# duxfrederic/lightcurver

Measured on AMD Instinct MI355X. Metric: cutouts/sec (PSF-fit + joint forward-model iter), 32x32 & 64x64 stamps, higher is better.
Workload: dtype f32

## Files before the change

lightcurver_amd/csrc/psf_kernels.h:

```cpp
#pragma once
#include <type_traits>
#include <utility>

#include "lc_common.h"
#include "starlet_device.h"

#ifndef LC_XPOLL_SLEEP
#define LC_XPOLL_SLEEP 2
#endif
#ifndef LC_P5_AHEAD
#define LC_P5_AHEAD 1
#endif
#ifndef LC_STARLET_LIVE_ADDR
#define LC_STARLET_LIVE_ADDR 1
#endif
namespace lc {
constexpr int kXFlagStride = 16;

#ifdef LC_STAMPS
__device__ long long g_stamps[128];
#define LC_STAMP(k)                                                      \
  do {                                                                   \
    if ((blockIdx.x == 0 || blockIdx.x == 8) && threadIdx.x == 0 && it == A.n_iter - 1)  \
      g_stamps[(k) + (blockIdx.x == 8 ? 64 : 0)] = clock64();            \
  } while (0)
#else
#define LC_STAMP(k) do {} while (0)
#endif


struct PsfArgs {
  int F, S, n_iter, t0, hist_stride, mode;
  const float *data, *wgt;
  const float *W;
  const float *norms;
  const float *Tm;
  float *B, *mB, *sB;
  float *stars, *stars_m, *stars_s;
  float *hist;
  float *qscratch;
  float *out_loss, *out_chi2, *out_gstars, *out_ggrid, *out_gT, *out_model;
  float lam_sc, lam_hf;
  lc_adabelief_cfg ab;
  float *xch;
  int *xflags, *xabort;
  int launch_seq, heal, force_abort_it;
  const float *bkB, *bkmB, *bksB, *bkstars, *bkstars_m, *bkstars_s;
  int *heal_count;
  const float *ext_grad;
  const float *sched;
  float *B1, *mB1, *sB1;
  int xcd_fast;
};

typedef float lc_v4f __attribute__((ext_vector_type(4)));
__device__ __forceinline__ void store_sc1_x4(float *p, lc_v4f v) {
  asm volatile("global_store_dwordx4 %0, %1, off sc1\n\ts_nop 2" ::"v"(p), "v"(v) : "memory");
}
__device__ __forceinline__ void store_plain_x4(float *p, lc_v4f v) {
  asm volatile("global_store_dwordx4 %0, %1, off\n\ts_nop 2" ::"v"(p), "v"(v) : "memory");
}
__device__ __forceinline__ void store_sc1_f(float *p, float v) {
  asm volatile("global_store_dword %0, %1, off sc1" ::"v"(p), "v"(v) : "memory");
}
__device__ __forceinline__ void load_sc1_2x4(const float *p, lc_v4f &a, lc_v4f &b) {
  asm volatile("global_load_dwordx4 %0, %2, off sc1\n\tglobal_load_dwordx4 %1, %2, off offset:16 sc1\n\ts_waitcnt vmcnt(0)"
               : "=&v"(a), "=&v"(b)
               : "v"(p)
               : "memory");
}
__device__ __forceinline__ void load_sc1_2x4_1(const float *p, lc_v4f &a, lc_v4f &b, const float *ps, float &s) {
  asm volatile("global_load_dword %2, %4, off sc1\n\tglobal_load_dwordx4 %0, %3, off sc1\n\tglobal_load_dwordx4 %1, %3, off offset:16 sc1\n\ts_waitcnt vmcnt(0)"
               : "=&v"(a), "=&v"(b), "=&v"(s)
               : "v"(p), "v"(ps)
               : "memory");
}
__device__ __forceinline__ void load_sc1_x4(const float *p, lc_v4f &a) {
  asm volatile("global_load_dwordx4 %0, %1, off sc1\n\ts_waitcnt vmcnt(0)" : "=&v"(a) : "v"(p) : "memory");
}
__device__ __forceinline__ float load_sc1_f(const float *p) {
  float v;
  asm volatile("global_load_dword %0, %1, off sc1\n\ts_waitcnt vmcnt(0)" : "=&v"(v) : "v"(p) : "memory");
  return v;
}


template <int N_, int SS_, int PX_, int SG_, bool WC_ = false, int JB_ = 8>
struct PsfCfg {
  static constexpr int N = N_, SS = SS_, PX = PX_, SG = SG_;
  static constexpr bool WC = WC_;
  static constexpr int n = N / SS;
  static constexpr int NTHR = N * N / PX;
  static constexpr int NW = (NTHR + kWave - 1) / kWave;
  static constexpr int NT = ntaps(SS);
  static constexpr int J = ilog2(N);
  static constexpr int LR = 8;
  static constexpr int LC = (JB_ * (N_ / SS_) / 4 >= 64) ? 4 : 2;
  static constexpr int LA = LC;
  static constexpr int TS = N + 1;
  static constexpr int RS = n + 1;
  static constexpr int OFF_T = 0;
  static constexpr int SZ_T = WC_ ? N * (N + 2 * (N / 4 + 10) + 1) : N * TS;
  static constexpr int OFF_R = OFF_T + SZ_T;
  static constexpr int SZ_R2 = SG * n * TS;
  static constexpr int VS = WC_ ? n + 3 : RS, VO = WC_ ? 1 : 0;
  static constexpr int SZ_V = SG * N * VS;
  static constexpr int JB = JB_;
  static constexpr int AP = N / 4 + 10;
  static constexpr int TSA = N + 2 * AP + 1;
  static constexpr int APR = AP / SS + 2;
  static constexpr int JBP = JB + 1;
  static constexpr int WSZ = JB * TSA + (n + 2 * APR) * JBP;
  static constexpr int SZ_VR = (SZ_V > StarletLds<N>::FLOATS) ? SZ_V : StarletLds<N>::FLOATS;
  static constexpr int OFF_WSC = OFF_R + SZ_VR;
  static constexpr int SZ_R = WC ? (SZ_VR + NW * WSZ) : ((2 * SZ_R2 > SZ_V) ? 2 * SZ_R2 : SZ_V);
  static constexpr int OFF_RES = OFF_R + SZ_R;
  static constexpr int SZ_RES = WC ? 0 : SG * n * n;
  static constexpr int OFF_TAPS = OFF_RES + SZ_RES;
  static constexpr int NTP = NT + 3;
  static constexpr int SZ_TAPS = (16 * 4 * NTP + 1) / 2 * 2 + 16 * 2 * NT * 2;
  static constexpr int OFF_TAPP = OFF_TAPS + (16 * 4 * NTP + 1) / 2 * 2;
  static constexpr int OFF_RED = OFF_TAPS + SZ_TAPS;
  static constexpr int IPS = n * n / LC;
  static constexpr int IPS_PAD = (IPS + kWave - 1) / kWave * kWave;
  static constexpr int SLOTS = IPS_PAD / kWave;
  static constexpr int SZ_REDX = 16 * NW;
  static constexpr int SZ_RED = (WC ? 16 * (n / JB) * 5 : SG * SLOTS * 5) + SZ_REDX + NW + 8;
  static constexpr int OFF_REDX = OFF_RED + (WC ? 16 * (n / JB) * 5 : SG * SLOTS * 5);
  static constexpr int OFF_REDW = OFF_REDX + SZ_REDX;
  static constexpr int OFF_STAR = OFF_RED + SZ_RED;
  static constexpr int MAXS = 16;
  static constexpr int SZ_STAR = MAXS * 20 + 16;
  static constexpr int LDS_FLOATS = OFF_STAR + SZ_STAR;
  static_assert(WC || StarletLds<N>::FLOATS <= SZ_T + SZ_R + SZ_RES, "starlet ping-pong buffers must fit over T + R + RES");
  static_assert(PX % SS == 0 && N % PX == 0 && n % LR == 0 && n % LC == 0 && n % LA == 0 && n % JB == 0, "tiling");
  static_assert(LDS_FLOATS * 4 <= 163840, "LDS");
  static_assert(OFF_TAPP % 2 == 0, "tap pairs are read as 64-bit words");
  static_assert(NTHR <= 1024 && NTHR % kWave == 0, "threads");
  static_assert(!WC_ || PX_ <= 8, "the WC layout keeps the pixel state in registers");
};


template <int SS, int NT>
__device__ inline void tap_entry(float delta, int k, float &tap, float &dtap, int &bq) {
  const int o = (int)nearbyintf(delta);
  const int base = o - kRg - (SS - 1);
  int q = base / SS;
  if (q * SS > base) --q;
  bq = q;
  const int m = q * SS + k;
  const float inv_s2 = 1.0f / (kSigmaG * kSigmaG);
  const float nrm = 0.3989422804014327f / kSigmaG;
  float a = 0.f, d = 0.f;
#pragma unroll
  for (int dv = 0; dv < SS; ++dv) {
    const int t = m + dv;
    if (t >= o - kRg && t <= o + kRg) {
      const float x = (float)t - delta;
      const float p = nrm * expf(-0.5f * x * x * inv_s2);
      a += p;
      d += p * x * inv_s2;
    }
  }
  tap = a;
  dtap = d;
}

template <class C, bool SPLIT = false>
__global__ __launch_bounds__(C::NTHR) void psf_fit_kernel(PsfArgs A) {
  constexpr int N = C::N, SS = C::SS, PX = C::PX, SG = C::SG, n = C::n, NT = C::NT, J = C::J;
  constexpr int NTHR = C::NTHR, TS = C::TS, RS = C::RS, LR = C::LR, LC = C::LC, LA = C::LA;
  extern __shared__ __align__(16) float lds[];
  float *T = lds + C::OFF_T;
  float *R2t = lds + C::OFF_R;
  float *R2xt = R2t + C::SZ_R2;
  float *V = lds + C::OFF_R;
  float *RES = lds + C::OFF_RES;
  float *TAPS = lds + C::OFF_TAPS + 1;
  constexpr int NTP = C::NTP;
  lc_v2f *TAPP = (lc_v2f *)(lds + C::OFF_TAPP);
  float *REDX = lds + C::OFF_REDX;
  float *RED = lds + C::OFF_RED;
  float *REDW = lds + C::OFF_REDW;
  float *SCAL = REDW + C::NW;
  float *SP = lds + C::OFF_STAR;
  float *SGR = SP + C::MAXS * 4;
  float *SM = SGR + C::MAXS * 5;
  float *SV = SM + C::MAXS * 4;
  int *BQ = (int *)(SV + C::MAXS * 4);

  int f = blockIdx.x, role = 0;
  if constexpr (SPLIT) {
    f = ((int)blockIdx.x >> 4) * 8 + ((int)blockIdx.x & 7);
    role = ((int)blockIdx.x >> 3) & 1;
    if (f >= A.F) return;
  }
  const bool conv_role = !SPLIT || role == 0, starlet_role = !SPLIT || role == 1;
  const int my_xcc = SPLIT ? (int)(__builtin_amdgcn_s_getreg(20 | (3 << 11)) & 15u) : 0;
  int same_xcd = 0;
  const int tid0 = threadIdx.x;
  const int S = A.S;

  const float *dataf = A.data + (size_t)f * S * n * n;
  const float *wgtf = A.wgt + (size_t)f * S * n * n;

  if constexpr (!SPLIT) {
    if (A.heal) {
      if (__hip_atomic_load(A.xabort, __ATOMIC_RELAXED, __HIP_MEMORY_SCOPE_AGENT) != A.launch_seq) return;
      const size_t o = (size_t)f * N * N;
      for (int i = tid0; i < N * N; i += NTHR) {
        A.B[o + i] = A.bkB[o + i];
        A.mB[o + i] = A.bkmB[o + i];
        A.sB[o + i] = A.bksB[o + i];
      }
      if (tid0 < S * 4) {
        A.stars[(size_t)f * S * 4 + tid0] = A.bkstars[(size_t)f * S * 4 + tid0];
        A.stars_m[(size_t)f * S * 4 + tid0] = A.bkstars_m[(size_t)f * S * 4 + tid0];
        A.stars_s[(size_t)f * S * 4 + tid0] = A.bkstars_s[(size_t)f * S * 4 + tid0];
      }
      if (f == 0 && tid0 == 0) atomicAdd(A.heal_count, 1);
      __threadfence_block();
      __syncthreads();
    }
  }

  if constexpr (C::WC) {
    for (int i = tid0; i < C::SZ_T; i += NTHR) lds[C::OFF_T + i] = 0.f;
    for (int i = tid0; i < C::NW * C::WSZ; i += NTHR) lds[C::OFF_WSC + i] = 0.f;
  }
  if (tid0 < S * 4) {
    SP[tid0] = A.stars[(size_t)f * S * 4 + tid0];
    SM[tid0] = A.stars_m[(size_t)f * S * 4 + tid0];
    SV[tid0] = A.stars_s[(size_t)f * S * 4 + tid0];
  }
  __syncthreads();

  constexpr bool STATE_REGS = (PX <= 8);
  float *Bg = A.B, *mBg = A.mB, *sBg = A.sB;
  if constexpr (SPLIT && !STATE_REGS) {
    if (role == 1) {
      const size_t g0pix = (size_t)f * N * N + (size_t)(tid0 / (N / PX)) * N + (tid0 % (N / PX)) * PX;
#pragma unroll
      for (int q = 0; q < PX / 4; ++q) {
        ((float4 *)(A.B1 + g0pix))[q] = ((const float4 *)(A.B + g0pix))[q];
        ((float4 *)(A.mB1 + g0pix))[q] = ((const float4 *)(A.mB + g0pix))[q];
        ((float4 *)(A.sB1 + g0pix))[q] = ((const float4 *)(A.sB + g0pix))[q];
      }
      Bg = A.B1;
      mBg = A.mB1;
      sBg = A.sB1;
    }
  }
  float Bp[PX], Mp[PX], Sp_[PX], Tp[PX];
  {
    const size_t g0pix = (size_t)f * N * N + (size_t)(tid0 / (N / PX)) * N + (tid0 % (N / PX)) * PX;
#pragma unroll
    for (int q = 0; q < PX / 4; ++q) {
      if (STATE_REGS) {
        const float4 b = ((const float4 *)(A.B + g0pix))[q], t = ((const float4 *)(A.Tm + g0pix))[q];
        const float4 m = ((const float4 *)(A.mB + g0pix))[q], sv = ((const float4 *)(A.sB + g0pix))[q];
        Bp[4 * q] = b.x; Bp[4 * q + 1] = b.y; Bp[4 * q + 2] = b.z; Bp[4 * q + 3] = b.w;
        Tp[4 * q] = t.x; Tp[4 * q + 1] = t.y; Tp[4 * q + 2] = t.z; Tp[4 * q + 3] = t.w;
        Mp[4 * q] = m.x; Mp[4 * q + 1] = m.y; Mp[4 * q + 2] = m.z; Mp[4 * q + 3] = m.w;
        Sp_[4 * q] = sv.x; Sp_[4 * q + 1] = sv.y; Sp_[4 * q + 2] = sv.z; Sp_[4 * q + 3] = sv.w;
      }
    }
  }

  auto compute_taps = [&](int tid) {
    for (int e = tid; e < S * 2 * NTP; e += NTHR) {
      const int s = e / (2 * NTP), ax = (e / NTP) & 1, k = e % NTP - 1;
      float tap = 0.f, dtap = 0.f;
      int bq = 0;
      const float c_off = (N % 2 == 0) ? 0.5f : 0.0f;
      const float delta = fminf(fmaxf(SS * SP[s * 4 + 1 + ax], -(float)(N / 4)), (float)(N / 4)) + c_off;
      if (k >= 0 && k < NT) tap_entry<SS, NT>(delta, k, tap, dtap, bq);
      TAPS[(s * 4 + 2 * ax) * NTP + k] = tap;
      TAPS[(s * 4 + 2 * ax + 1) * NTP + k] = dtap;
      if (k >= 0 && k < NT) TAPP[(s * 2 + ax) * NT + k] = (lc_v2f){tap, dtap};
      if (k == 0) BQ[s * 2 + ax] = bq;
    }
  };
  auto step_stars = [&](int tid) {
#pragma clang fp contract(off)
    if (tid < S * 3) {
      const float lr = SCAL[0], bc1 = SCAL[1], bc2 = SCAL[2];
      const float b1 = A.ab.b1, b2 = A.ab.b2, eps = A.ab.eps, eps_root = A.ab.eps_root;
      const int s = tid / 3, q = tid % 3;
      const float g = SGR[s * 5 + 1 + q];
      const float mn = b1 * SM[s * 4 + q] + (1.f - b1) * g;
      const float dg = g - mn;
      const float sn = b2 * SV[s * 4 + q] + (1.f - b2) * dg * dg + eps_root;
      SM[s * 4 + q] = mn;
      SV[s * 4 + q] = sn;
      SP[s * 4 + q] -= lr * (mn * bc1) / (sqrtf(sn * bc2) + eps);
    }
  };
  auto update_stars_and_taps = [&](int tid) {
    step_stars(tid);
    __syncthreads();
    compute_taps(tid);
  };
  if (conv_role) compute_taps(tid0);
  for (int it = 0; it < A.n_iter; ++it) {
    const int tglob = A.t0 + it;
    if constexpr (SPLIT) {
      if (A.force_abort_it == it && f == 0 && role == 1) {
        if (tid0 == 0) __hip_atomic_store(A.xabort, A.launch_seq, __ATOMIC_RELAXED, __HIP_MEMORY_SCOPE_AGENT);
        break;
      }
    }
    int tid = tid0;
    LC_LAUNDER(tid);
    const int lane = tid & 63, wid = tid >> 6;
    const int pu = tid / (N / PX);
    const int pv = (tid % (N / PX)) * PX;
    const size_t gpix = (size_t)f * N * N + (size_t)pu * N + pv;
    if (tid < 3 && A.mode == 1) SCAL[tid] = A.sched[3 * tglob + tid];
    LC_STAMP(0);
    float gB[PX];
#pragma unroll
    for (int p = 0; p < PX; ++p) gB[p] = 0.f;
    float tpix[PX];
    if (conv_role) {
    if (C::WC && STATE_REGS) {
#pragma unroll
      for (int p = 0; p < PX; ++p) {
        tpix[p] = Bp[p] + Tp[p];
        T[pu * C::TSA + C::AP + pv + p] = tpix[p];
      }
    } else if (STATE_REGS) {
#pragma unroll
      for (int p = 0; p < PX; ++p) T[pu * TS + pv + p] = Bp[p] + Tp[p];
    } else {
      const float4 *bp = (const float4 *)(Bg + gpix);
      const float4 *tp = (const float4 *)(A.Tm + gpix);
#pragma unroll
      for (int q = 0; q < PX / 4; ++q) {
        const float4 b = bp[q], t = tp[q];
        T[pu * TS + pv + 4 * q + 0] = b.x + t.x;
        T[pu * TS + pv + 4 * q + 1] = b.y + t.y;
        T[pu * TS + pv + 4 * q + 2] = b.z + t.z;
        T[pu * TS + pv + 4 * q + 3] = b.w + t.w;
      }
    }
    if (tid < S * 5) SGR[tid] = 0.f;

    for (int g0 = 0; g0 < S; g0 += SG) {
      __syncthreads();
      LC_STAMP(1 + 5 * (g0 / SG));
      if constexpr (C::WC) {
        constexpr int JB = C::JB, NBLK = n / JB;
        float *wsc = lds + C::OFF_WSC + wid * C::WSZ;
        constexpr int TSA = C::TSA, AP = C::AP, APR = C::APR;
        float *R2w = wsc + AP, *RESw = wsc + JB * TSA + APR * C::JBP;
        int kdone = 0;
        for (int task = wid; task < SG * NBLK; task += C::NW, ++kdone) {
          progress_prio(kdone);
          const int sl = task / NBLK, blk = task % NBLK, s = g0 + sl;
          if (s >= S) continue;
          const int jd0 = blk * JB;
          const float *tx = TAPS + (s * 4 + 0) * NTP, *ty = tx + 2 * NTP, *dty = tx + 3 * NTP;
          const int bqx = BQ[s * 2 + 0], bqy = BQ[s * 2 + 1];
          const float amp = SP[s * 4 + 0], sky = SP[s * 4 + 3];
          constexpr int NI3 = (JB * (n / LC) + 63) / 64;
          float dpre[NI3][LC], wpre[NI3][LC];
#pragma unroll
          for (int i3 = 0; i3 < NI3; ++i3) {
            const int item = lane + 64 * i3;
            const bool ok = item < JB * (n / LC);
            const int jl = item % JB, a0 = (item / JB) * LC;
#pragma unroll
            for (int j = 0; j < LC; ++j) {
              const size_t pix = ok ? ((size_t)s * n * n + (size_t)(a0 + j) * n + jd0 + jl) : 0;
              const float dv = dataf[pix], wv = wgtf[pix];
              dpre[i3][j] = ok ? dv : 0.f;
              wpre[i3][j] = ok ? wv : 0.f;
            }
          }
          LC_STAMP(10);
          {
            const int ws = SS * (jd0 - bqx) - (NT - 1);
            if constexpr (SS == 2) {
              constexpr int NP = (NT + 1) / 2, WL2 = (JB - 1) + NP;
              lc_v2f tr2[NP];
#pragma unroll
              for (int h = 0; h < NP; ++h) tr2[h] = (lc_v2f){tx[NT - 1 - 2 * h], tx[NT - 2 - 2 * h]};
              for (int u = lane; u < N; u += 64) {
                lc_v2f win2[WL2];
                const float *trow = T + u * TSA + AP + ws;
#pragma unroll
                for (int i = 0; i < WL2; ++i) win2[i] = (lc_v2f){trow[2 * i], trow[2 * i + 1]};
                lc_v2f acc[JB];
#pragma unroll
                for (int j = 0; j < JB; ++j) acc[j] = (lc_v2f){0.f, 0.f};
#pragma unroll
                for (int h = 0; h < NP; ++h) {
#pragma unroll
                  for (int j = 0; j < JB; ++j) acc[j] = pk_fma(tr2[h], win2[j + h], acc[j]);
                }
#pragma unroll
                for (int j = 0; j < JB; ++j) R2w[j * TSA + u] = acc[j].x + acc[j].y;
              }
            } else {
              constexpr int WL = SS * (JB - 1) + NT;
              float tk[NT];
#pragma unroll
              for (int k = 0; k < NT; ++k) tk[k] = tx[k];
              for (int u = lane; u < N; u += 64) {
                float win[WL];
                const float *trow = T + u * TSA + AP + ws;
#pragma unroll
                for (int i = 0; i < WL; ++i) win[i] = trow[i];
#pragma unroll
                for (int j = 0; j < JB; ++j) {
                  float acc = 0.f;
#pragma unroll
                  for (int k = 0; k < NT; ++k) acc = fmaf(tk[k], win[SS * j - k + NT - 1], acc);
                  R2w[j * TSA + u] = acc;
                }
              }
            }
          }
          wave_lds_sync();
          LC_STAMP(11);
          float chi = 0.f, ga = 0.f, gy = 0.f, gs = 0.f;
          {
            constexpr int WL = SS * (LC - 1) + NT;
            lc_v2f tyd[NT];
#pragma unroll
            for (int k = 0; k < NT; ++k) tyd[k] = TAPP[(s * 2 + 1) * NT + k];
#pragma unroll
            for (int i3 = 0; i3 < NI3; ++i3) {
              const int item = lane + 64 * i3;
              if (item < JB * (n / LC)) {
                const int jl = item % JB, a0 = (item / JB) * LC;
                const int ws = SS * (a0 - bqy) - (NT - 1);
                float win[WL];
                const float *r2 = R2w + jl * TSA + ws;
#pragma unroll
                for (int i = 0; i < WL; ++i) win[i] = r2[i];
                float lgy = 0.f;
                lc_v2f fvys[LC];
#pragma unroll
                for (int j = 0; j < LC; ++j) fvys[j] = (lc_v2f){0.f, 0.f};
#pragma unroll
                for (int k = 0; k < NT; ++k) {
#pragma unroll
                  for (int j = 0; j < LC; ++j) fvys[j] = pk_fma(tyd[k], pk_bcast(win[SS * j - k + NT - 1]), fvys[j]);
                  if constexpr (LC == 4) asm volatile("" : "+v"(fvys[0]), "+v"(fvys[1]), "+v"(fvys[2]), "+v"(fvys[3]));
                  else asm volatile("" : "+v"(fvys[0]), "+v"(fvys[1]));
                }
#pragma unroll
                for (int j = 0; j < LC; ++j) {
                  const float fv = fvys[j].x, fy = fvys[j].y;
                  const float model = fmaf(amp, fv, sky);
                  const float res = model - dpre[i3][j];
                  const float rw = wpre[i3][j] * res;
                  chi = fmaf(rw, res, chi);
                  ga = fmaf(rw, fv, ga);
                  lgy = fmaf(rw, fy, lgy);
                  gs += rw;
                  RESw[(a0 + j) * C::JBP + jl] = rw;
                  if (A.out_model) A.out_model[(size_t)f * S * n * n + (size_t)s * n * n + (size_t)(a0 + j) * n + jd0 + jl] = model;
                }
                gy += lgy * amp * SS;
              }
            }
          }
          wave_sum4(chi, ga, gy, gs);
          if (lane == 0) {
            float *r = RED + (s * NBLK + blk) * 5;
            r[0] = chi;
            r[1] = ga;
            r[3] = gy;
            r[4] = gs;
          }
          wave_lds_sync();
          LC_STAMP(12);
          {
            constexpr int WI = (SS * LA - 1 + NT - 1) / SS + 1;
            constexpr int NI4 = (JB * (n / LA) + 63) / 64;
            if constexpr (SS == 2) {
              constexpr int NP = (NT + 1) / 2;
              lc_v2f py[NP];
#pragma unroll
              for (int q = 0; q < NP; ++q) py[q] = (lc_v2f){ty[2 * q], ty[2 * q - 1]};
#pragma unroll
              for (int i4 = 0; i4 < NI4; ++i4) {
                const int item = lane + 64 * i4;
                if (item < JB * (n / LA)) {
                  const int jl = item % JB, a0 = (item / JB) * LA;
                  lc_v2f out2[LA];
#pragma unroll
                  for (int h = 0; h < LA; ++h) out2[h] = (lc_v2f){0.f, 0.f};
                  const float *rcol = RESw + (bqy + a0) * C::JBP + jl;
#pragma unroll
                  for (int i = 0; i < WI; ++i) {
                    const lc_v2f rv = pk_bcast(rcol[i * C::JBP]);
#pragma unroll
                    for (int h = 0; h < LA; ++h)
                      if (i - h >= 0 && i - h < NP) out2[h] = pk_fma(py[i - h], rv, out2[h]);
                  }
                  float *vrow = V + (sl * N + SS * a0) * C::VS + C::VO + jd0 + jl;
#pragma unroll
                  for (int h = 0; h < LA; ++h) {
                    vrow[(2 * h) * C::VS] = out2[h].x;
                    vrow[(2 * h + 1) * C::VS] = out2[h].y;
                  }
                  if (jd0 + jl == 0) {
#pragma unroll
                    for (int r = 0; r < SS * LA; ++r) V[(sl * N + SS * a0 + r) * C::VS] = 0.f;
                  }
                  if (jd0 + jl == n - 1) {
#pragma unroll
                    for (int r = 0; r < SS * LA; ++r) V[(sl * N + SS * a0 + r) * C::VS + n + 1] = 0.f;
                  }
                }
              }
            } else {
              float tk[NT];
#pragma unroll
              for (int k = 0; k < NT; ++k) tk[k] = ty[k];
#pragma unroll
              for (int i4 = 0; i4 < NI4; ++i4) {
                const int item = lane + 64 * i4;
                if (item < JB * (n / LA)) {
                  const int jl = item % JB, a0 = (item / JB) * LA;
                  float out[SS * LA];
#pragma unroll
                  for (int r = 0; r < SS * LA; ++r) out[r] = 0.f;
                  const float *rcol = RESw + (bqy + a0) * C::JBP + jl;
#pragma unroll
                  for (int i = 0; i < WI; ++i) {
                    const float rv = rcol[i * C::JBP];
#pragma unroll
                    for (int k = 0; k < NT; ++k) {
                      const int rel = SS * i - k;
                      if (rel >= 0 && rel < SS * LA) out[rel] = fmaf(tk[k], rv, out[rel]);
                    }
                  }
#pragma unroll
                  for (int r = 0; r < SS * LA; ++r) V[(sl * N + SS * a0 + r) * C::VS + C::VO + jd0 + jl] = out[r];
                  if (jd0 + jl == 0) {
#pragma unroll
                    for (int r = 0; r < SS * LA; ++r) V[(sl * N + SS * a0 + r) * C::VS] = 0.f;
                  }
                  if (jd0 + jl == n - 1) {
#pragma unroll
                    for (int r = 0; r < SS * LA; ++r) V[(sl * N + SS * a0 + r) * C::VS + n + 1] = 0.f;
                  }
                }
              }
            }
          }
          wave_lds_sync();
          LC_STAMP(13);
        }
        __builtin_amdgcn_s_setprio(0);
        LC_STAMP(14);
#ifdef LC_STAMPS
        if (blockIdx.x == 0 && lane == 0 && it == A.n_iter - 1) g_stamps[20 + wid] = clock64();
#endif
        __syncthreads();
        LC_STAMP(15);
        if (tid < SG * 5) {
          const int sl = tid / 5, q = tid % 5;
          if (g0 + sl < S && q != 2) {
            float acc = 0.f;
            for (int k = 0; k < NBLK; ++k) acc += RED[((g0 + sl) * NBLK + k) * 5 + q];
            SGR[(g0 + sl) * 5 + q] = acc;
          }
        }
      } else {
      constexpr int NIT3 = (SG * C::IPS_PAD + NTHR - 1) / NTHR;
      float dpre[NIT3][LC], wpre[NIT3][LC];
#pragma unroll
      for (int i3 = 0; i3 < NIT3; ++i3) {
        const int item0 = wid * 64 + i3 * NTHR, item = item0 + lane;
        const int sl = item0 / C::IPS_PAD, within = item % C::IPS_PAD, s = g0 + sl;
        const bool ok = (item0 < SG * C::IPS_PAD) && (s < S) && (within < C::IPS);
        const int jd = within % n, a0 = (within / n) * LC;
#pragma unroll
        for (int j = 0; j < LC; ++j) {
          const size_t pix = ok ? ((size_t)s * n * n + (size_t)(a0 + j) * n + jd) : 0;
          const float dv = dataf[pix], wv = wgtf[pix];
          dpre[i3][j] = ok ? dv : 0.f;
          wpre[i3][j] = ok ? wv : 0.f;
        }
      }
      {
        constexpr int WL = SS * (LR - 1) + NT;
        constexpr int NSTRIP = n / LR;
        for (int item = tid; item < SG * N * NSTRIP; item += NTHR) {
          const int u = item % N, strip = (item / N) % NSTRIP, sl = item / (N * NSTRIP);
          if (g0 + sl >= S) continue;
          const float *tx = TAPS + ((g0 + sl) * 4 + 0) * NTP;
          const int bq = BQ[(g0 + sl) * 2 + 0];
          const int a0 = strip * LR;
          const int ws = SS * (a0 - bq) - (NT - 1);
          float win[WL];
#pragma unroll
          for (int i = 0; i < WL; ++i) {
            const int idx = ws + i;
            const int ci = min(max(idx, 0), N - 1);
            const float v = T[u * TS + ci];
            win[i] = (idx >= 0 && idx < N) ? v : 0.f;
          }
          float tk[NT];
#pragma unroll
          for (int k = 0; k < NT; ++k) tk[k] = tx[k];
#pragma unroll
          for (int j = 0; j < LR; ++j) {
            float acc = 0.f;
#pragma unroll
            for (int k = 0; k < NT; ++k) acc = fmaf(tk[k], win[SS * j - k + NT - 1], acc);
            R2t[(sl * n + a0 + j) * TS + u] = acc;
          }
        }
      }
      __syncthreads();
      LC_STAMP(2 + 5 * (g0 / SG));
      {
        constexpr int WL = SS * (LC - 1) + NT;
        constexpr int NSTRIP = n / LC;
#pragma unroll
        for (int i3 = 0; i3 < NIT3; ++i3) {
          const int item0 = wid * 64 + i3 * NTHR;
          if (item0 >= SG * C::IPS_PAD) break;
          const int item = item0 + lane;
          const int sl = item0 / C::IPS_PAD;
          const int within = item % C::IPS_PAD;
          const int s = g0 + sl;
          float chi = 0.f, ga = 0.f, gx = 0.f, gy = 0.f, gs = 0.f;
          if (s < S && within < C::IPS) {
            const int jd = within % n, strip = within / n;
            const float *ty = TAPS + (s * 4 + 2) * NTP, *dty = ty + NTP;
            const int bq = BQ[s * 2 + 1];
            const int a0 = strip * LC;
            const int ws = SS * (a0 - bq) - (NT - 1);
            const float amp = SP[s * 4 + 0], sky = SP[s * 4 + 3];
            float win[WL];
#pragma unroll
            for (int i = 0; i < WL; ++i) {
              const int idx = ws + i;
              const int ci = min(max(idx, 0), N - 1);
              const bool ok = (idx >= 0 && idx < N);
              const float v = R2t[(sl * n + jd) * TS + ci];
              win[i] = ok ? v : 0.f;
            }
            float tk[NT], dk[NT];
#pragma unroll
            for (int k = 0; k < NT; ++k) {
              tk[k] = ty[k];
              dk[k] = dty[k];
            }
#pragma unroll
            for (int j = 0; j < LC; ++j) {
              float fv = 0.f, fy = 0.f;
#pragma unroll
              for (int k = 0; k < NT; ++k) {
                const float w = win[SS * j - k + NT - 1];
                fv = fmaf(tk[k], w, fv);
                fy = fmaf(dk[k], w, fy);
              }
              const int id = a0 + j;
              const size_t pix = (size_t)s * n * n + (size_t)id * n + jd;
              const float d = dpre[i3][j], w = wpre[i3][j];
              const float model = fmaf(amp, fv, sky);
              const float res = model - d;
              const float rw = w * res;
              chi = fmaf(rw, res, chi);
              ga = fmaf(rw, fv, ga);
              gy = fmaf(rw, fy, gy);
              gs += rw;
              RES[(sl * n + id) * n + jd] = rw;
              if (A.out_model) A.out_model[(size_t)f * S * n * n + pix] = model;
            }
            gy *= amp * SS;
          }
          chi = wave_sum(chi);
          ga = wave_sum(ga);
          gx = wave_sum(gx);
          gy = wave_sum(gy);
          gs = wave_sum(gs);
          if (lane == 0) {
            float *r = RED + (sl * C::SLOTS + (item0 % C::IPS_PAD) / 64) * 5;
            r[0] = chi;
            r[1] = ga;
            r[2] = gx;
            r[3] = gy;
            r[4] = gs;
          }
        }
      }
      __syncthreads();
      LC_STAMP(3 + 5 * (g0 / SG));
      if (tid < SG * 5) {
        const int sl = tid / 5, q = tid % 5;
        if (g0 + sl < S && q != 2) {
          float acc = 0.f;
          for (int k = 0; k < C::SLOTS; ++k) acc += RED[(sl * C::SLOTS + k) * 5 + q];
          SGR[(g0 + sl) * 5 + q] = acc;
        }
      }
      {
        constexpr int WI = (SS * LA - 1 + NT - 1) / SS + 1;
        constexpr int NSTRIP = n / LA;
        for (int item = tid; item < SG * n * NSTRIP; item += NTHR) {
          const int jd = item % n, strip = (item / n) % NSTRIP, sl = item / (n * NSTRIP);
          if (g0 + sl >= S) continue;
          const float *ty = TAPS + ((g0 + sl) * 4 + 2) * NTP;
          const int bq = BQ[(g0 + sl) * 2 + 1];
          const int a0 = strip * LA;
          float tk[NT];
#pragma unroll
          for (int k = 0; k < NT; ++k) tk[k] = ty[k];
          float out[SS * LA];
#pragma unroll
          for (int r = 0; r < SS * LA; ++r) out[r] = 0.f;
#pragma unroll
          for (int i = 0; i < WI; ++i) {
            const int id = i + bq + a0;
            const int ci = min(max(id, 0), n - 1);
            float rv = RES[(sl * n + ci) * n + jd];
            rv = (id >= 0 && id < n) ? rv : 0.f;
#pragma unroll
            for (int k = 0; k < NT; ++k) {
              const int rel = SS * i - k;
              if (rel >= 0 && rel < SS * LA) out[rel] = fmaf(tk[k], rv, out[rel]);
            }
          }
#pragma unroll
          for (int r = 0; r < SS * LA; ++r) V[(sl * N + SS * a0 + r) * RS + jd] = out[r];
        }
      }
      __syncthreads();
      LC_STAMP(4 + 5 * (g0 / SG));
      }
      LC_STAMP(16);
      if constexpr (C::WC) {
        constexpr int WJ = (PX - 1 + NT - 1) / SS + 1;
        constexpr bool AHEAD = SPLIT && PX == 8 && LC_P5_AHEAD;
        if constexpr (AHEAD) {
          static_assert(SG % 8 == 0, "two stars per turn of the loop share a priority step");
          struct P5Ops {
            float vwin[WJ];
            lc_v2f txd[NT];
            float amp;
          };
          auto p5_star = [&](int sl, const P5Ops &use, auto on_the_way) {
            const int s = g0 + sl;
            lc_v2f accp[PX];
#pragma unroll
            for (int p = 0; p < PX; ++p) accp[p] = (lc_v2f){0.f, 0.f};
#pragma unroll
            for (int i = 0; i < WJ; ++i) {
              if (i == 4) on_the_way();
              const lc_v2f vv = pk_bcast(use.vwin[i]);
#pragma unroll
              for (int k = 0; k < NT; ++k) {
                const int rel = SS * i - k;
                if (rel >= 0 && rel < PX) accp[rel] = pk_fma(use.txd[k], vv, accp[rel]);
              }
            }
            float gxs = 0.f;
#pragma unroll
            for (int p = 0; p < PX; ++p) {
              gB[p] = fmaf(use.amp, accp[p].x, gB[p]);
              gxs = fmaf(accp[p].y, tpix[p], gxs);
            }
            gxs = wave_sum(gxs);
            if (lane == 0) REDX[s * C::NW + wid] = gxs;
          };
          auto nothing = [] {};
          auto p5_window = [&](int sl, P5Ops &o, int bq) {
            o.amp = SP[(g0 + sl) * 4 + 0];
            const float *vrow = V + (sl * N + pu) * C::VS + 1;
            const int jd0 = bq + pv / SS;
#pragma unroll
            for (int i = 0; i < WJ; ++i) o.vwin[i] = vrow[min(max(jd0 + i, -1), n)];
            __builtin_amdgcn_sched_barrier(0);
          };
          auto p5_taps = [&](int sl, P5Ops &o) {
            __builtin_amdgcn_sched_barrier(0);
#pragma unroll
            for (int k = 0; k < NT; ++k) o.txd[k] = TAPP[((g0 + sl) * 2 + 0) * NT + k];
            __builtin_amdgcn_sched_barrier(0);
          };
          const int ns = min(SG, S - g0);
          P5Ops opsA, opsB;
          int bqn = BQ[min(g0 + 1, S - 1) * 2 + 0];
          p5_window(0, opsA, BQ[g0 * 2 + 0]);
          p5_taps(0, opsA);
          int sl = 0;
#pragma clang loop unroll(disable)
          while (sl + 1 < ns) {
            progress_prio((4 * sl) / SG);
            const int bqnn = BQ[min(g0 + sl + 2, S - 1) * 2 + 0];
            p5_window(sl + 1, opsB, bqn);
            p5_star(sl, opsA, [&] { p5_taps(sl + 1, opsB); });
            if (sl + 2 >= ns) {
              opsA = opsB;
              sl += 1;
              break;
            }
            bqn = BQ[min(g0 + sl + 3, S - 1) * 2 + 0];
            p5_window(sl + 2, opsA, bqnn);
            p5_star(sl + 1, opsB, [&] { p5_taps(sl + 2, opsA); });
            sl += 2;
          }
          progress_prio((4 * sl) / SG);
          p5_star(sl, opsA, nothing);
        } else {
          for (int sl = 0; sl < SG; ++sl) {
            const int s = g0 + sl;
            if (s >= S) break;
            progress_prio((4 * sl) / SG);
            const int bq = BQ[s * 2 + 0];
            const float amp = SP[s * 4 + 0];
            lc_v2f txd[NT];
#pragma unroll
            for (int k = 0; k < NT; ++k) txd[k] = TAPP[(s * 2 + 0) * NT + k];
            lc_v2f accp[PX];
#pragma unroll
            for (int p = 0; p < PX; ++p) accp[p] = (lc_v2f){0.f, 0.f};
            const float *vrow = V + (sl * N + pu) * C::VS + 1;
            const int jd0 = bq + pv / SS;
            float vwin[WJ];
#pragma unroll
            for (int i = 0; i < WJ; ++i) vwin[i] = vrow[min(max(jd0 + i, -1), n)];
#pragma unroll
            for (int i = 0; i < WJ; ++i) {
              const lc_v2f vv = pk_bcast(vwin[i]);
#pragma unroll
              for (int k = 0; k < NT; ++k) {
                const int rel = SS * i - k;
                if (rel >= 0 && rel < PX) accp[rel] = pk_fma(txd[k], vv, accp[rel]);
              }
            }
            float gxs = 0.f;
#pragma unroll
            for (int p = 0; p < PX; ++p) {
              gB[p] = fmaf(amp, accp[p].x, gB[p]);
              gxs = fmaf(accp[p].y, tpix[p], gxs);
            }
            gxs = wave_sum(gxs);
            if (lane == 0) REDX[s * C::NW + wid] = gxs;
          }
        }
        __builtin_amdgcn_s_setprio(0);
      } else {
        constexpr int WJ = (PX - 1 + NT - 1) / SS + 1;
        for (int sl = 0; sl < SG; ++sl) {
          const int s = g0 + sl;
          if (s >= S) break;
          const float *tx = TAPS + (s * 4 + 0) * NTP, *dtx = tx + NTP;
          const int bq = BQ[s * 2 + 0];
          const float amp = SP[s * 4 + 0];
          float acc[PX], gxs = 0.f;
#pragma unroll
          for (int p = 0; p < PX; ++p) acc[p] = 0.f;
#pragma unroll
          for (int i = 0; i < WJ; ++i) {
            const int jd = i + bq + pv / SS;
            const int ci = min(max(jd, 0), n - 1);
            float vv = V[(sl * N + pu) * RS + ci];
            vv = (jd >= 0 && jd < n) ? vv : 0.f;
            float dsum = 0.f;
#pragma unroll
            for (int k = 0; k < NT; ++k) {
              const int rel = SS * i - k;
              if (rel >= 0 && rel < PX) {
                acc[rel] = fmaf(tx[k], vv, acc[rel]);
                dsum = fmaf(dtx[k], T[pu * TS + pv + rel], dsum);
              }
            }
            gxs = fmaf(vv, dsum, gxs);
          }
#pragma unroll
          for (int p = 0; p < PX; ++p) gB[p] = fmaf(amp, acc[p], gB[p]);
          gxs = wave_sum(gxs);
          if (lane == 0) REDX[s * C::NW + wid] = gxs;
        }
      }
      LC_STAMP(17);
    }
    if (A.ext_grad) {
#pragma unroll
      for (int p = 0; p < PX; ++p) gB[p] += A.ext_grad[gpix + p];
    }
    }
    __syncthreads();
    LC_STAMP(40);
    {
      if (conv_role && tid < S) {
        float acc = 0.f;
#pragma unroll
        for (int w = 0; w < C::NW; ++w) acc += REDX[tid * C::NW + w];
        SGR[tid * 5 + 2] = acc * SP[tid * 4 + 0] * SS;
      }
    }

    if (A.out_gT) {
#pragma unroll
      for (int p = 0; p < PX; ++p) A.out_gT[gpix + p] = gB[p];
    }

    float l1 = 0.f;
    float z[PX];
#pragma unroll
    for (int p = 0; p < PX; ++p) z[p] = 0.f;
    if (starlet_role && (A.lam_sc != 0.f || A.lam_hf != 0.f)) {
      float bpix[PX];
      if (STATE_REGS) {
#pragma unroll
        for (int p = 0; p < PX; ++p) bpix[p] = Bp[p];
      } else {
        const float4 *bp = (const float4 *)(Bg + gpix);
#pragma unroll
        for (int q = 0; q < PX / 4; ++q) {
          const float4 b = bp[q];
          bpix[4 * q] = b.x;
          bpix[4 * q + 1] = b.y;
          bpix[4 * q + 2] = b.z;
          bpix[4 * q + 3] = b.w;
        }
      }
      constexpr bool LIVE_ADDR = SPLIT && STATE_REGS && LC_STARLET_LIVE_ADDR;
      starlet_l1_grad<N, PX, ilog2(N), LIVE_ADDR>(bpix, A.W ? A.W + (size_t)f * J * N * N : nullptr, A.norms,
                                                  A.qscratch + (size_t)f * J * N * N, A.lam_sc, A.lam_hf,
                                                  C::WC ? lds + C::OFF_R : lds, tid, l1, z);
    }
    LC_STAMP(42);
    {
      const float wl = wave_sum(l1);
      if (lane == 0) REDW[wid] = wl;
    }
    __syncthreads();
    float tl1 = 0.f;
    if (tid == 0 && starlet_role)
      for (int w = 0; w < C::NW; ++w) tl1 += REDW[w];
    LC_STAMP(44);
    if constexpr (SPLIT) {
      constexpr int XS = N * N + 64;
      float *mine = A.xch + (((size_t)f * 2 + (it & 1)) * 2 + role) * XS;
      const float *theirs = A.xch + (((size_t)f * 2 + (it & 1)) * 2 + (1 - role)) * XS;
      const int poff = pu * N + pv;
#pragma unroll
      for (int q = 0; q < PX / 4; ++q) {
        lc_v4f v;
        v.x = role ? z[4 * q] : gB[4 * q];
        v.y = role ? z[4 * q + 1] : gB[4 * q + 1];
        v.z = role ? z[4 * q + 2] : gB[4 * q + 2];
        v.w = role ? z[4 * q + 3] : gB[4 * q + 3];
        if (same_xcd) store_plain_x4(mine + poff + 4 * q, v);
        else store_sc1_x4(mine + poff + 4 * q, v);
      }
      if (tid == 0 && role == 1) {
        if (same_xcd) asm volatile("global_store_dword %0, %1, off" ::"v"(mine + N * N), "v"(tl1) : "memory");
        else store_sc1_f(mine + N * N, tl1);
      }
      if (tid == 0 && it == 0) store_sc1_f(mine + N * N + 1, __int_as_float(my_xcc + 1));
      constexpr bool TAPS_LATE = STATE_REGS;
      if (role == 0 && A.mode == 1) {
        if (TAPS_LATE) step_stars(tid);
        else update_stars_and_taps(tid);
      }
      asm volatile("s_waitcnt vmcnt(0)" ::: "memory");
      __syncthreads();
      LC_STAMP(45);
      int *OK = (int *)(SCAL + 5);
      if (tid == 0) {
        if (same_xcd) asm volatile("global_store_dword %0, %1, off" ::"v"(A.xflags + ((size_t)f * 2 + role) * kXFlagStride), "v"(it + 1) : "memory");
        else __hip_atomic_store(A.xflags + ((size_t)f * 2 + role) * kXFlagStride, it + 1, __ATOMIC_RELAXED, __HIP_MEMORY_SCOPE_AGENT);
        int ok = 1, spins = 0;
        while (__hip_atomic_load(A.xflags + ((size_t)f * 2 + (1 - role)) * kXFlagStride, __ATOMIC_RELAXED, __HIP_MEMORY_SCOPE_AGENT) < it + 1) {
          __builtin_amdgcn_s_sleep(LC_XPOLL_SLEEP);
          ++spins;
          if (spins > (1 << 21) ||
              ((spins & 255) == 0 && __hip_atomic_load(A.xabort, __ATOMIC_RELAXED, __HIP_MEMORY_SCOPE_AGENT) == A.launch_seq)) {
            __hip_atomic_store(A.xabort, A.launch_seq, __ATOMIC_RELAXED, __HIP_MEMORY_SCOPE_AGENT);
            ok = 0;
            break;
          }
        }
        if (it == 0 && ok) OK[1] = (A.xcd_fast && __float_as_int(load_sc1_f(theirs + N * N + 1)) == my_xcc + 1) ? 1 : 0;
        *OK = ok;
#ifdef LC_XCH_ACQUIRE
        __builtin_amdgcn_fence(__ATOMIC_ACQUIRE, "agent");
        asm volatile("s_waitcnt vmcnt(0)" ::: "memory");
#endif
      }
      if (TAPS_LATE && role == 0 && A.mode == 1) compute_taps((tid + NTHR / 2) % NTHR);
      __syncthreads();
      LC_STAMP(46);
      if (*OK == 0) break;
      if (it == 0) same_xcd = OK[1];
      float other[PX];
      float tl1_other = 0.f;
      if constexpr (PX == 8) {
        lc_v4f a, b;
        load_sc1_2x4_1(theirs + poff, a, b, theirs + N * N, tl1_other);
        other[0] = a.x; other[1] = a.y; other[2] = a.z; other[3] = a.w;
        other[4] = b.x; other[5] = b.y; other[6] = b.z; other[7] = b.w;
      } else {
#pragma unroll
        for (int q = 0; q < PX / 4; ++q) {
          lc_v4f a;
          load_sc1_x4(theirs + poff + 4 * q, a);
          other[4 * q] = a.x; other[4 * q + 1] = a.y; other[4 * q + 2] = a.z; other[4 * q + 3] = a.w;
        }
      }
#pragma unroll
      for (int p = 0; p < PX; ++p) {
        if (role) gB[p] = other[p]; else z[p] = other[p];
      }
      if (tid == 0 && role == 0) tl1 = (PX == 8) ? tl1_other : load_sc1_f(theirs + N * N);
      LC_STAMP(47);
    }
    if (tid == 0 && conv_role) {
      float chi = 0.f;
      for (int s = 0; s < S; ++s) chi += SGR[s * 5];
      const float loss = 0.5f * chi + tl1;
      A.hist[(size_t)f * A.hist_stride + tglob] = loss;
      if (A.out_loss) A.out_loss[f] = loss;
      if (A.out_chi2) A.out_chi2[f] = chi;
    }
    if (A.out_ggrid) {
#pragma unroll
      for (int p = 0; p < PX; ++p) A.out_ggrid[gpix + p] = gB[p] + z[p];
    }
    if (A.out_gstars && tid < S * 4) {
      const int s = tid / 4, q = tid % 4;
      A.out_gstars[(size_t)f * S * 4 + tid] = SGR[s * 5 + 1 + q];
    }
    if (A.mode == 1) {
#pragma clang fp contract(off)
      const float lr = SCAL[0], bc1 = SCAL[1], bc2 = SCAL[2];
      const float b1 = A.ab.b1, b2 = A.ab.b2, eps = A.ab.eps, eps_root = A.ab.eps_root;
      if (STATE_REGS) {
#pragma unroll
        for (int p = 0; p < PX; ++p) {
          const float g = gB[p] + z[p];
          const float mn = b1 * Mp[p] + (1.f - b1) * g;
          const float dg = g - mn;
          const float sn = b2 * Sp_[p] + (1.f - b2) * dg * dg + eps_root;
          Mp[p] = mn;
          Sp_[p] = sn;
          Bp[p] -= lr * (mn * bc1) * __builtin_amdgcn_rcpf(__builtin_amdgcn_sqrtf(sn * bc2) + eps);
        }
      }
      if constexpr (!STATE_REGS) {
        float4 *bp = (float4 *)(Bg + gpix);
        float4 *mp = (float4 *)(mBg + gpix);
        float4 *sp = (float4 *)(sBg + gpix);
        float4 bq[PX / 4], mq[PX / 4], sq[PX / 4];
#pragma unroll
        for (int q = 0; q < PX / 4; ++q) {
          bq[q] = bp[q];
          mq[q] = mp[q];
          sq[q] = sp[q];
        }
#pragma unroll
        for (int q = 0; q < PX / 4; ++q) {
          float *bb = &bq[q].x, *mm = &mq[q].x, *ss_ = &sq[q].x;
#pragma unroll
          for (int e = 0; e < 4; ++e) {
            const float g = gB[4 * q + e] + z[4 * q + e];
            const float mn = b1 * mm[e] + (1.f - b1) * g;
            const float dg = g - mn;
            const float sn = b2 * ss_[e] + (1.f - b2) * dg * dg + eps_root;
            mm[e] = mn;
            ss_[e] = sn;
            bb[e] -= lr * (mn * bc1) * __builtin_amdgcn_rcpf(__builtin_amdgcn_sqrtf(sn * bc2) + eps);
          }
        }
#pragma unroll
        for (int q = 0; q < PX / 4; ++q) {
          bp[q] = bq[q];
          mp[q] = mq[q];
          sp[q] = sq[q];
        }
      }
      if constexpr (!SPLIT) update_stars_and_taps(tid);
    }
    __syncthreads();
    LC_STAMP(43);
  }

  if (A.mode == 1 && STATE_REGS && conv_role) {
    const size_t g0pix = (size_t)f * N * N + (size_t)(tid0 / (N / PX)) * N + (tid0 % (N / PX)) * PX;
#pragma unroll
    for (int q = 0; q < PX / 4; ++q) {
      ((float4 *)(A.B + g0pix))[q] = make_float4(Bp[4 * q], Bp[4 * q + 1], Bp[4 * q + 2], Bp[4 * q + 3]);
      ((float4 *)(A.mB + g0pix))[q] = make_float4(Mp[4 * q], Mp[4 * q + 1], Mp[4 * q + 2], Mp[4 * q + 3]);
      ((float4 *)(A.sB + g0pix))[q] = make_float4(Sp_[4 * q], Sp_[4 * q + 1], Sp_[4 * q + 2], Sp_[4 * q + 3]);
    }
  }
  if (A.mode == 1 && tid0 < S * 4 && conv_role) {
    A.stars[(size_t)f * S * 4 + tid0] = SP[tid0];
    A.stars_m[(size_t)f * S * 4 + tid0] = SM[tid0];
    A.stars_s[(size_t)f * S * 4 + tid0] = SV[tid0];
  }
}

}
```

Baseline: 58.83 million.

## Trim serial barriers in split conv/starlet iteration by prefetching next T and early exchange store

```diff
diff --git a/lightcurver_amd/csrc/psf_kernels.h b/lightcurver_amd/csrc/psf_kernels.h
--- a/lightcurver_amd/csrc/psf_kernels.h
+++ b/lightcurver_amd/csrc/psf_kernels.h
@@ -13,6 +13,9 @@
 #endif
 #ifndef LC_STARLET_LIVE_ADDR
 #define LC_STARLET_LIVE_ADDR 1
+#endif
+#ifndef LC_SERIAL_TRIM
+#define LC_SERIAL_TRIM 1
 #endif
 namespace lc {
 constexpr int kXFlagStride = 16;
@@ -302,6 +305,20 @@
     compute_taps(tid);
   };
   if (conv_role) compute_taps(tid0);
+  constexpr bool TRIM = SPLIT && C::WC && PX == 8 && LC_SERIAL_TRIM;
+  static_assert(!TRIM || 3 * C::MAXS <= kWave, "the x0 sums and the stars' step are lanes of one wave");
+  [[maybe_unused]] float tpix_next[TRIM ? PX : 1];
+  if constexpr (TRIM) {
+    if (role == 0) {
+      const int pu = tid0 / (N / PX), pv = (tid0 % (N / PX)) * PX;
+#pragma unroll
+      for (int p = 0; p < PX; ++p) {
+        tpix_next[p] = Bp[p] + Tp[p];
+        T[pu * C::TSA + C::AP + pv + p] = tpix_next[p];
+      }
+    }
+    __syncthreads();
+  }
   for (int it = 0; it < A.n_iter; ++it) {
     const int tglob = A.t0 + it;
     if constexpr (SPLIT) {
@@ -323,7 +340,10 @@
     for (int p = 0; p < PX; ++p) gB[p] = 0.f;
     float tpix[PX];
     if (conv_role) {
-    if (C::WC && STATE_REGS) {
+    if constexpr (TRIM) {
+#pragma unroll
+      for (int p = 0; p < PX; ++p) tpix[p] = tpix_next[p];
+    } else if (C::WC && STATE_REGS) {
 #pragma unroll
       for (int p = 0; p < PX; ++p) {
         tpix[p] = Bp[p] + Tp[p];
@@ -347,7 +367,7 @@
     if (tid < S * 5) SGR[tid] = 0.f;
 
     for (int g0 = 0; g0 < S; g0 += SG) {
-      __syncthreads();
+      if (!TRIM || g0 > 0) __syncthreads();
       LC_STAMP(1 + 5 * (g0 / SG));
       if constexpr (C::WC) {
         constexpr int JB = C::JB, NBLK = n / JB;
@@ -891,6 +911,23 @@
       for (int p = 0; p < PX; ++p) gB[p] += A.ext_grad[gpix + p];
     }
     }
+    if constexpr (TRIM) {
+      if (role == 0) {
+        LC_STAMP(41);
+        float *mine = A.xch + (((size_t)f * 2 + (it & 1)) * 2 + 0) * (N * N + 64);
+#pragma unroll
+        for (int q = 0; q < PX / 4; ++q) {
+          lc_v4f v;
+          v.x = gB[4 * q];
+          v.y = gB[4 * q + 1];
+          v.z = gB[4 * q + 2];
+          v.w = gB[4 * q + 3];
+          if (same_xcd) store_plain_x4(mine + pu * N + pv + 4 * q, v);
+          else store_sc1_x4(mine + pu * N + pv + 4 * q, v);
+        }
+        if (tid == 0 && it == 0) store_sc1_f(mine + N * N + 1, __int_as_float(my_xcc + 1));
+      }
+    }
     __syncthreads();
     LC_STAMP(40);
     {
@@ -933,11 +970,13 @@
                                                   C::WC ? lds + C::OFF_R : lds, tid, l1, z);
     }
     LC_STAMP(42);
-    {
-      const float wl = wave_sum(l1);
-      if (lane == 0) REDW[wid] = wl;
-    }
-    __syncthreads();
+    if (!TRIM || role == 1) {
+      {
+        const float wl = wave_sum(l1);
+        if (lane == 0) REDW[wid] = wl;
+      }
+      __syncthreads();
+    }
     float tl1 = 0.f;
     if (tid == 0 && starlet_role)
       for (int w = 0; w < C::NW; ++w) tl1 += REDW[w];
@@ -947,6 +986,7 @@
       float *mine = A.xch + (((size_t)f * 2 + (it & 1)) * 2 + role) * XS;
       const float *theirs = A.xch + (((size_t)f * 2 + (it & 1)) * 2 + (1 - role)) * XS;
       const int poff = pu * N + pv;
+      if (!TRIM || role == 1) {
 #pragma unroll
       for (int q = 0; q < PX / 4; ++q) {
         lc_v4f v;
@@ -962,8 +1002,10 @@
         else store_sc1_f(mine + N * N, tl1);
       }
       if (tid == 0 && it == 0) store_sc1_f(mine + N * N + 1, __int_as_float(my_xcc + 1));
+      }
       constexpr bool TAPS_LATE = STATE_REGS;
       if (role == 0 && A.mode == 1) {
+        if constexpr (TRIM) wave_lds_sync();
         if (TAPS_LATE) step_stars(tid);
         else update_stars_and_taps(tid);
       }
@@ -1019,7 +1061,7 @@
       if (tid == 0 && role == 0) tl1 = (PX == 8) ? tl1_other : load_sc1_f(theirs + N * N);
       LC_STAMP(47);
     }
-    if (tid == 0 && conv_role) {
+    if (!TRIM && tid == 0 && conv_role) {
       float chi = 0.f;
       for (int s = 0; s < S; ++s) chi += SGR[s * 5];
       const float loss = 0.5f * chi + tl1;
@@ -1085,6 +1127,23 @@
       }
       if constexpr (!SPLIT) update_stars_and_taps(tid);
     }
+    if constexpr (TRIM) {
+      if (role == 0) {
+#pragma unroll
+        for (int p = 0; p < PX; ++p) {
+          tpix_next[p] = Bp[p] + Tp[p];
+          T[pu * C::TSA + C::AP + pv + p] = tpix_next[p];
+        }
+        if (tid == 0) {
+          float chi = 0.f;
+          for (int s = 0; s < S; ++s) chi += SGR[s * 5];
+          const float loss = 0.5f * chi + tl1;
+          A.hist[(size_t)f * A.hist_stride + tglob] = loss;
+          if (A.out_loss) A.out_loss[f] = loss;
+          if (A.out_chi2) A.out_chi2[f] = chi;
+        }
+      }
+    }
     __syncthreads();
     LC_STAMP(43);
   }
```

After: 60.34 million, median of 6. 2.6% higher.
